# cropinghigh/sdrpp-dvbs-demodulator

Hardware: NVIDIA B200
Metric: decoded_info_gbit_s (higher is better)
Workload: dtype int8

## Files before the change

### sdrpp-dvbs-demodulator_b200/csrc/ldpc_decoder.cuh

```cuda
#pragma once
#include <cstdint>
#include <cuda_runtime.h>

namespace s2 {

constexpr int kLdpcThreads = 384;
constexpr int kBitWords = 13;
constexpr int16_t kLdpcItersNoInput = -2;

struct LdpcPlan;

struct LdpcDev {
    int N, K, R, q;
    int ngroups;
    int max_cnt;
    int sg;
    bool chains;
    bool occ3;
    bool v2;
    bool lanes2;
    const LdpcPlan* plan;
    const uint32_t* links;
    const int* layer_off;
    const uint8_t* layer_nlev;
    const uint8_t* row_level;
};
int ldpc_slot_groups(int max_cnt);
bool ldpc_chains_pay_off(int code_index);
bool ldpc_ctas_wanted3(int code_index);
bool ldpc_use_v2(int code_index);
bool ldpc_use_lanes2(int code_index);
int ldpc_slot_groups_for(int max_cnt, bool lanes2);
int ldpc_prepare(LdpcDev& code);
void ldpc_release(LdpcDev& code);

struct LdpcArgs {
    LdpcDev code;
    const int8_t* llr_in;
    int nframes;
    int max_trials;
    uint8_t* hard_out;
    int hard_stride;
    int16_t* iters_out;
    int8_t* llr_out;
    uint8_t* workspace;
    unsigned int* work_counter;
    const unsigned int* arrived;
};

inline size_t ldpc_workspace_bytes(const LdpcDev& c) {
    size_t b = (size_t)c.q * c.sg * 360 * 16 + (((size_t)c.R * 2 + 15) & ~(size_t)15);
    if (c.v2) b += (size_t)2 * (c.ngroups + c.q) * kBitWords * 4 + 32 + (size_t)768 * 16;
    return (b + 255) & ~(size_t)255;
}
inline size_t ldpc_smem_bytes(const LdpcDev& c) {
    if (c.v2 && c.lanes2) return (size_t)c.K * 2 + 768 + (size_t)c.q * (4 + 2 * ((2 * ((c.max_cnt + 1) / 2) + 3) & ~3)) * 4 + 64;
    if (c.v2) return (size_t)c.K * 2 + 768 + (size_t)c.q * ((1 + 2 * c.max_cnt + 3) & ~3) * 4 + 64;
    const size_t base = (size_t)c.K * 2 + (size_t)2 * (c.ngroups + c.q) * kBitWords * 4;
    return c.chains ? ((base + 15) & ~(size_t)15) + 360 * 16 + 64 : base + 64;
}

int ldpc_launch(const LdpcArgs& args, int grid, cudaStream_t stream);
int ldpc_max_ctas_per_sm(const LdpcDev& code);

}
```

### sdrpp-dvbs-demodulator_b200/csrc/ldpc_v2.cuh

```cuda
#pragma once
#include "ldpc_decoder.cuh"
#include "ldpc_variants.h"

#include <type_traits>

namespace s2 {
namespace v2 {

constexpr int kThreads = 360;

__device__ __forceinline__ uint32_t prmt(uint32_t a, uint32_t b, uint32_t sel) {
    uint32_t d;
    asm("prmt.b32 %0, %1, %2, %3;" : "=r"(d) : "r"(a), "r"(b), "r"(sel));
    return d;
}
__device__ __forceinline__ uint32_t minu2(uint32_t a, uint32_t b) {
    uint32_t d;
    asm("min.u16x2 %0, %1, %2;" : "=r"(d) : "r"(a), "r"(b));
    return d;
}
__device__ __forceinline__ uint32_t min3u2(uint32_t a, uint32_t b, uint32_t c) {
    uint32_t d;
    asm("{.reg .b32 t; min.u16x2 t, %1, %2; min.u16x2 %0, t, %3;}" : "=r"(d) : "r"(a), "r"(b), "r"(c));
    return d;
}
__device__ __forceinline__ uint32_t addmin_relu(uint32_t a, uint32_t b, uint32_t c) {
    uint32_t d;
    asm("{.reg .b32 t; add.s16x2 t, %1, %2; min.s16x2.relu %0, t, %3;}" : "=r"(d) : "r"(a), "r"(b), "r"(c));
    return d;
}
__device__ __forceinline__ uint32_t addmin(uint32_t a, uint32_t b, uint32_t c) {
    uint32_t d;
    asm("{.reg .b32 t; add.s16x2 t, %1, %2; min.s16x2 %0, t, %3;}" : "=r"(d) : "r"(a), "r"(b), "r"(c));
    return d;
}
__device__ __forceinline__ uint32_t addmin_u32(uint32_t x, uint32_t c) {
    uint32_t d;
    asm("{.reg .b32 t; add.u32 t, %1, %2; min.u32 %0, t, %1;}" : "=r"(d) : "r"(x), "r"(c));
    return d;
}
__device__ __forceinline__ uint32_t lds_u16(uint32_t addr) {
    uint16_t v;
    asm volatile("ld.shared.u16 %0, [%1];" : "=h"(v) : "r"(addr));
    return v;
}
__device__ __forceinline__ uint32_t lds_u32(uint32_t addr) {
    uint32_t v;
    asm volatile("ld.shared.u32 %0, [%1];" : "=r"(v) : "r"(addr));
    return v;
}
__device__ __forceinline__ void sts_u16(uint32_t addr, uint32_t v) {
    asm volatile("st.shared.u16 [%0], %1;" ::"r"(addr), "h"((uint16_t)v));
}

__device__ __forceinline__ uint32_t unpack_lo(uint32_t w) { return prmt(w, 0, 0x4140); }
__device__ __forceinline__ uint32_t unpack_hi(uint32_t w) { return prmt(w, 0, 0x4342); }
__device__ __forceinline__ uint32_t pack_pair(uint32_t x) { return prmt(x, 0, 0x4420); }
__device__ __forceinline__ uint32_t pack_two(uint32_t x0, uint32_t x1) { return prmt(x0, x1, 0x6420); }
__device__ __forceinline__ uint32_t lane_mask7(uint32_t x) { return prmt(x, 0, 0xAA88); }

constexpr uint32_t kC128 = 0x00800080u, kC255 = 0x00FF00FFu, kM32 = 0xFFE0FFE0u, kP32 = 0x00200020u;
constexpr uint32_t kP63 = 0x003F003Fu, kP64 = 0x00400040u, kAllOnes = 0xFFFFFFFFu;

template <int D>
__device__ __forceinline__ void exclusive_min(const uint32_t (&a)[D], uint32_t (&ex)[D]) {
    static_assert(D >= 3, "a check has at least three links");
    uint32_t P[D], S[D + 2];
#pragma unroll
    for (int i = 1; i < D; i += 2) P[i] = (i == 1) ? minu2(a[0], a[1]) : min3u2(P[i - 2], a[i - 1], a[i]);
    constexpr int top = (D & 1) ? D - 1 : D - 2;
    S[top] = (D & 1) ? a[D - 1] : minu2(a[D - 2], a[D - 1]);
#pragma unroll
    for (int i = top - 2; i >= 0; i -= 2) S[i] = min3u2(a[i], a[i + 1], S[i + 2]);
#pragma unroll
    for (int k = 0; k < D; ++k) {
        uint32_t t[4];
        int n = 0;
        if (k & 1) {
            if (k >= 3) t[n++] = P[k - 2];
            t[n++] = a[k - 1];
        } else if (k >= 2) {
            t[n++] = P[k - 1];
        }
        if (k + 1 <= D - 1) {
            if (((k + 1) & 1) == 0 && k + 1 <= top) {
                t[n++] = S[k + 1];
            } else {
                t[n++] = a[k + 1];
                if (k + 2 <= top) t[n++] = S[k + 2];
            }
        }
        ex[k] = (n == 1) ? t[0] : (n == 2) ? minu2(t[0], t[1]) : min3u2(t[0], t[1], t[2]);
    }
}

template <int CNT, bool FIRST, bool RAGGED>
__device__ __forceinline__ void row_update(const uint32_t (&off)[CNT], int cnt, uint32_t (&mw)[(CNT + 3) / 2],
                                           uint32_t& pown, uint32_t& psec, uint32_t keep, uint32_t m1) {
    constexpr int D = CNT + 2;
    uint32_t tu[D], a[D], ex[D];
    uint32_t sx = ((D - 1) & 1) ? kC128 : 0u;
#pragma unroll
    for (int c = 0; c < D; ++c) {
        uint32_t u;
        if (c < CNT)
            u = (!RAGGED || c < cnt) ? unpack_lo(lds_u16(off[c])) : kC255;
        else
            u = (c == CNT) ? pown : psec;
        uint32_t t = u;
        if (!FIRST) {
            const uint32_t beta = (c & 1) ? unpack_hi(mw[c >> 1]) : unpack_lo(mw[c >> 1]);
            t = addmin_relu(u + beta, kM32, kC255);
        }
        tu[c] = t;
        a[c] = __vabsdiffu4(t, kC128);
        sx ^= t;
    }
    exclusive_min<D>(a, ex);
    const uint32_t ssx = lane_mask7(sx);
    uint32_t prev = 0;
#pragma unroll
    for (int c = 0; c < D; ++c) {
        const uint32_t om = addmin_relu(ex[c], kAllOnes, kP32);
        const uint32_t neg = lane_mask7(tu[c]) ^ ssx;
        const uint32_t bias = neg * 0xFFFEFFFFu + kP32;
        const uint32_t bm = addmin(om ^ neg, bias, kP63);
        const uint32_t un = addmin_relu(tu[c] + bm, kM32, kC255);
        uint32_t beta;
        asm("mad.lo.u32 %0, %1, %2, %3;" : "=r"(beta) : "r"(bm), "r"(m1), "r"(kP64));
        if (c < CNT) {
            if (!RAGGED || c < cnt) sts_u16(off[c], pack_pair(un));
        } else if (c == CNT) {
            pown = un;
        } else {
            psec = un;
        }
        if (c & 1)
            mw[c >> 1] = pack_two(prev, beta);
        else if (c == D - 1)
            mw[c >> 1] = prmt(beta, keep, 0x7620);
        prev = beta;
    }
}


__device__ __forceinline__ uint32_t win360(const uint32_t* H, int o) {
    int w = o >> 5, s = o & 31;
    uint32_t r = __funnelshift_r(__ldcg(H + w), __ldcg(H + w + 1), s);
    int over = o + 32 - 360;
    if (over > 0) r |= __ldcg(H) << (32 - over);
    return r;
}
__device__ __forceinline__ uint32_t harvest8(uint4 w, uint32_t& nzacc) {
    const uint32_t k80 = 0x80808080u;
    nzacc &= __vabsdiffu4(w.x, k80) + 0x7F7F7F7Fu;
    nzacc &= __vabsdiffu4(w.y, k80) + 0x7F7F7F7Fu;
    nzacc &= __vabsdiffu4(w.z, k80) + 0x7F7F7F7Fu;
    nzacc &= __vabsdiffu4(w.w, k80) + 0x7F7F7F7Fu;
    uint32_t a0 = prmt(w.x, w.y, 0x6420), b0 = prmt(w.x, w.y, 0x7531);
    uint32_t a1 = prmt(w.z, w.w, 0x6420), b1 = prmt(w.z, w.w, 0x7531);
    auto mask4 = [](uint32_t x) { return (((~x & 0x80808080u) >> 7) * 0x00204081u >> 21) & 0xFu; };
    return mask4(a0) | (mask4(a1) << 4) | (mask4(b0) << 8) | (mask4(b1) << 12);
}
template <bool GLOBAL, int THREADS>
__device__ __forceinline__ void harvest_planes(const uint4* src, int n360, uint32_t* H, int gstride, int tid,
                                               uint32_t& nzacc) {
    uint8_t* Hb = reinterpret_cast<uint8_t*>(H);
    for (int t = tid; t < n360 * 45; t += THREADS) {
        uint4 w = GLOBAL ? __ldcg(src + t) : src[t];
        uint32_t bits = harvest8(w, nzacc);
        int g = t / 45, k = t - g * 45;
        __stcg(&Hb[g * (kBitWords * 4) + k], (uint8_t)bits);
        __stcg(&Hb[(gstride + g) * (kBitWords * 4) + k], (uint8_t)(bits >> 8));
    }
}

template <int THREADS>
__device__ __noinline__ int full_test(const LdpcParams2& p, const uint16_t* wpty, uint32_t* HP, uint32_t* HD,
                                      const uint4* vdata4, int* s_bad) {
    const int tid = threadIdx.x, q = p.q;
    uint32_t nzacc = 0xFFFFFFFFu;
    harvest_planes<true, THREADS>(reinterpret_cast<const uint4*>(wpty), q, HP, q, tid, nzacc);
    harvest_planes<false, THREADS>(vdata4, p.ngroups, HD, p.ngroups, tid, nzacc);
    if (tid < 2) s_bad[tid] = 0;
    __syncthreads();
    if (~nzacc & 0x00800080u) atomicOr(&s_bad[0], 1);
    if (~nzacc & 0x80008000u) atomicOr(&s_bad[1], 1);
    for (int task = tid; task < q * 12; task += THREADS) {
        const int ii = task / 12, w = task - ii * 12;
        const int loff = p.layer_off[ii], cnt = (int)p.layer_off[ii + 1] - loff;
        uint32_t sA = __ldcg(&HP[ii * kBitWords + w]), sB = __ldcg(&HP[(q + ii) * kBitWords + w]);
        if (ii > 0) {
            sA ^= __ldcg(&HP[(ii - 1) * kBitWords + w]);
            sB ^= __ldcg(&HP[(q + ii - 1) * kBitWords + w]);
        } else {
            const uint32_t* ta = &HP[(q - 1) * kBitWords];
            const uint32_t* tb = &HP[(2 * q - 1) * kBitWords];
            sA ^= (__ldcg(ta + w) << 1) | (w ? __ldcg(ta + w - 1) >> 31 : 0u);
            sB ^= (__ldcg(tb + w) << 1) | (w ? __ldcg(tb + w - 1) >> 31 : 0u);
        }
        for (int c = 0; c < cnt; ++c) {
            int o = 32 * w + (int)(p.link_add[loff + c] >> 1) - 360;
            o += (o < 0) ? 360 : 0;
            const int g = p.link_group[loff + c];
            sA ^= win360(&HD[g * kBitWords], o);
            sB ^= win360(&HD[(p.ngroups + g) * kBitWords], o);
        }
        if (w == 11) {
            sA &= 0xFFu;
            sB &= 0xFFu;
        }
        if (sA) atomicOr(&s_bad[0], 1);
        if (sB) atomicOr(&s_bad[1], 1);
    }
    __syncthreads();
    return (s_bad[0] ? 1 : 0) | (s_bad[1] ? 2 : 0);
}

template <int THREADS>
__device__ __noinline__ void emit_results(const LdpcParams2& p, int fin, const int (&res)[2], int fa, int fb,
                                          const uint16_t* wpty, const uint4* vdata4) {
    const int tid = threadIdx.x, q = p.q, K = p.K, N = p.N, R = p.R;
    const int kbytes = K / 8;
    for (int b = tid; b < kbytes; b += THREADS) {
        uint32_t nz = 0xFFFFFFFFu;
        const uint32_t bits = harvest8(vdata4[b], nz);
        if (fin & 1) p.hard_out[(size_t)fa * p.hard_stride + b] = (uint8_t)(__brev(bits & 0xFFu) >> 24);
        if (fin & 2) p.hard_out[(size_t)fb * p.hard_stride + b] = (uint8_t)(__brev((bits >> 8) & 0xFFu) >> 24);
    }
    for (int f = 0; f < 2; ++f) {
        if (!(fin >> f & 1)) continue;
        const int fr = f ? fb : fa;
        if (tid == 0) p.iters_out[fr] = (int16_t)res[f];
        if (p.llr_out) {
            int8_t* lo = p.llr_out + (size_t)fr * N;
            const uint8_t* vb = reinterpret_cast<const uint8_t*>(vdata4) + f;
            for (int x = tid; x < K; x += THREADS) lo[x] = (int8_t)(vb[2 * x] ^ 0x80u);
            for (int x = tid; x < R; x += THREADS) {
                const int jj = x / q, ii = x - jj * q;
                lo[K + x] = (int8_t)((__ldcg(&wpty[360 * ii + jj]) >> (8 * f)) ^ 0x80u);
            }
        }
    }
}

__device__ __forceinline__ uint4 interleave8(uint2 a, uint2 b) {
    uint4 o;
    o.x = prmt(a.x, b.x, 0x5140) ^ 0x80808080u;
    o.y = prmt(a.x, b.x, 0x7362) ^ 0x80808080u;
    o.z = prmt(a.y, b.y, 0x5140) ^ 0x80808080u;
    o.w = prmt(a.y, b.y, 0x7362) ^ 0x80808080u;
    return o;
}
template <bool STREAMED>
__device__ __forceinline__ uint2 ld_in8(const int8_t* frame, int x) {
    const uint2* s = reinterpret_cast<const uint2*>(frame) + x;
    return STREAMED ? __ldcg(s) : __ldg(s);
}

template <bool STREAMED, int THREADS>
__device__ __noinline__ void load_pair(const LdpcParams2& p, const int8_t* inA, const int8_t* inB, uint16_t* vdata,
                                       uint16_t* wpty) {
    static_assert(THREADS % 360 == 0, "a whole number of threads per column");
    const int tid = threadIdx.x, q = p.q, K = p.K;
    uint4* v4 = reinterpret_cast<uint4*>(vdata);
    const int8_t* ptA = inA + K;
    const int8_t* ptB = inB + K;
    const int cols = min(360, (K / q) & ~7);
    const int jj = tid % 360, i0 = tid / 360;
    for (int j0 = 0; j0 < 360; j0 += cols) {
        const int nc = min(cols, 360 - j0);
        const int b8 = q * j0 / 8;
        for (int x = tid; x < q * nc / 8; x += THREADS) v4[x] = interleave8(ld_in8<STREAMED>(ptA, b8 + x), ld_in8<STREAMED>(ptB, b8 + x));
        __syncthreads();
        if (jj < nc)
            for (int i = i0; i < q; i += THREADS / 360) __stcg(&wpty[i * 360 + j0 + jj], vdata[jj * q + i]);
        __syncthreads();
    }
    for (int x = tid; x < K / 8; x += THREADS) v4[x] = interleave8(ld_in8<STREAMED>(inA, x), ld_in8<STREAMED>(inB, x));
}

constexpr unsigned kNoPair = 0xFFFFFFFFu;
template <bool STREAMED>
__device__ __noinline__ unsigned claim_next_pair(const LdpcParams2& p, unsigned npairs) {
    if (*reinterpret_cast<const volatile unsigned*>(p.work_counter) + gridDim.x >= npairs) return kNoPair;
    const unsigned np = atomicAdd(p.work_counter, 1u);
    if (np < npairs) {
        const unsigned f0 = 2u * np, nf = min(2u, (unsigned)p.nframes - f0);
        if (!STREAMED || *reinterpret_cast<const volatile unsigned*>(p.arrived) >= f0 + nf) {
            const size_t b = reinterpret_cast<size_t>(p.llr_in + (size_t)f0 * p.N);
            const size_t lo = b & ~(size_t)15, hi = (b + (size_t)nf * p.N + 15) & ~(size_t)15;
            asm volatile("cp.async.bulk.prefetch.L2.global [%0], %1;" ::"l"(lo), "r"((unsigned)(hi - lo)) : "memory");
        }
    }
    return np;
}

static __device__ __noinline__ bool wait_arrived(const unsigned int* arrived_ptr, unsigned need, long long budget) {
    const volatile unsigned* arrived = arrived_ptr;
    const long long t0 = clock64();
    while (*arrived < need) {
        __nanosleep(500);
        if (clock64() - t0 > budget) return false;
    }
    return true;
}

template <int CNT, bool RAGGED, bool STREAMED, int OCC>
__global__ void __launch_bounds__(kThreads, OCC) ldpc_v2_kernel(const __grid_constant__ LdpcParams2 p) {
    constexpr int SLOTS = CNT + 2;
    constexpr int MW = (SLOTS + 1) / 2;
    constexpr int SG = (SLOTS + 7) / 8;
    static_assert(16 * SG >= 2 * SLOTS + 2, "the message record needs two spare bytes (row level)");
    constexpr int DW = (1 + 2 * CNT + 3) & ~3;
    extern __shared__ __align__(16) uint8_t smem_raw[];
    const int q = p.q, K = p.K, N = p.N, R = p.R;
    uint16_t* vdata = reinterpret_cast<uint16_t*>(smem_raw);
    uint16_t* X = reinterpret_cast<uint16_t*>(smem_raw + (size_t)K * 2);
    uint32_t* desc = reinterpret_cast<uint32_t*>(smem_raw + (size_t)K * 2 + 768);
    __shared__ unsigned int s_pair;
    __shared__ int s_bad[2];

    const int tid = threadIdx.x;
    const int j = tid;
    const uint32_t vbase = (uint32_t)__cvta_generic_to_shared(vdata);
    uint32_t dbase = (uint32_t)__cvta_generic_to_shared(desc);
    uint32_t j2 = 2u * (uint32_t)j;
    uint32_t xaddr = (uint32_t)__cvta_generic_to_shared(X) + j2;
    uint32_t m1 = 0xFFFFFFFFu;
    uint4* wmsg = reinterpret_cast<uint4*>(p.workspace + (size_t)blockIdx.x * p.ws_stride);
    uint16_t* wpty = reinterpret_cast<uint16_t*>(p.workspace + (size_t)blockIdx.x * p.ws_stride + (size_t)q * SG * 360 * 16);
    uint32_t* HD = reinterpret_cast<uint32_t*>(reinterpret_cast<uint8_t*>(wpty) + (((size_t)R * 2 + 15) & ~(size_t)15));
    uint32_t* HP = HD + 2 * p.ngroups * kBitWords;
    {
        volatile uint4* opq = reinterpret_cast<volatile uint4*>(HP + 2 * q * kBitWords + 4) + tid;
        opq->x = j2; opq->y = xaddr; opq->z = dbase; opq->w = m1;
        j2 = opq->x; xaddr = opq->y; dbase = opq->z; m1 = opq->w;
    }
    for (int x = tid; x < q * DW; x += kThreads) {
        const int i = x / DW, w = x - i * DW;
        const int loff = p.layer_off[i], cnt = (int)p.layer_off[i + 1] - loff;
        uint32_t v = 0;
        if (w == 0) {
            v = (uint32_t)p.layer_nlev[i] | (uint32_t)p.layer_sync[i] << 8 | (uint32_t)cnt << 16;
        } else if (w <= 2 * CNT) {
            const int c = (w - 1) >> 1;
            const int k = loff + (c < cnt ? c : 0);
            v = ((w - 1) & 1) ? (uint32_t)p.link_add[k] : vbase + 720u * p.link_group[k];
        }
        desc[x] = v;
    }
    const int npairs = (p.nframes + 1) >> 1;

    for (int x = tid; x < 2 * (p.ngroups + q) * kBitWords; x += kThreads) __stcg(&HD[x], 0u);
    __shared__ unsigned int s_next;
    if (tid == 0) s_next = kNoPair;

    for (;;) {
        __syncthreads();
        if (tid == 0) {
            unsigned np = s_next;
            if (np == kNoPair) np = atomicAdd(p.work_counter, 1u);
            s_next = kNoPair;
            if (STREAMED && np < (unsigned)npairs) {
                if (!wait_arrived(p.arrived, min(2u * np + 2u, (unsigned)p.nframes), p.wait_budget)) np |= 0x80000000u;
                __threadfence();
            }
            s_pair = np;
        }
        __syncthreads();
        const unsigned pair_word = s_pair;
        const unsigned pair = pair_word & 0x7FFFFFFFu;
        if (pair >= (unsigned)npairs) break;
        const int fa = 2 * pair, fb = 2 * pair + 1;
        const bool hasB = fb < p.nframes;
        if (STREAMED && (pair_word & 0x80000000u)) {
            if (tid == 0) {
                p.iters_out[fa] = kLdpcItersNoInput;
                if (hasB) p.iters_out[fb] = kLdpcItersNoInput;
            }
            continue;
        }
        const int8_t* inA = p.llr_in + (size_t)fa * N;
        const int8_t* inB = p.llr_in + (size_t)(hasB ? fb : fa) * N;

        load_pair<STREAMED, kThreads>(p, inA, inB, vdata, wpty);
        uint32_t pown = 0, psec = 0;
        {
            const uint32_t last = __ldcg(wpty + (q - 1) * 360 + j);
            X[j + 1] = (uint16_t)last;
            pown = unpack_lo(last);
            psec = unpack_lo(__ldcg(wpty + (q - 2) * 360 + j));
        }
        if (tid == 0) X[0] = 0xFFFFu;

        int live = hasB ? 3 : 1;
        uint32_t off[CNT];
        uint32_t lw0 = 0;
        auto link_addresses = [&](int i) {
            uint32_t dw[DW];
#pragma unroll
            for (int x = 0; x < DW; x += 4)
                asm volatile("ld.shared.v4.u32 {%0, %1, %2, %3}, [%4];" : "=r"(dw[x]), "=r"(dw[x + 1]), "=r"(dw[x + 2]), "=r"(dw[x + 3])
                             : "r"(dbase + (uint32_t)(i * DW + x) * 4u));
            lw0 = dw[0];
#pragma unroll
            for (int c = 0; c < CNT; ++c)
                off[c] = dw[1 + 2 * c] + addmin_u32(j2 + dw[2 + 2 * c], (uint32_t)-720);
        };
        auto screen = [&]() -> int {
            link_addresses(q - 1);
            const int cnt = (int)(lw0 >> 16);
            uint32_t sx = pown ^ psec, mn = minu2(__vabsdiffu4(pown, kC128), __vabsdiffu4(psec, kC128));
            int nl = 2;
#pragma unroll
            for (int c = 0; c < CNT; ++c) {
                if (!RAGGED || c < cnt) {
                    const uint32_t u = unpack_lo(lds_u16(off[c]));
                    sx ^= u;
                    mn = minu2(mn, __vabsdiffu4(u, kC128));
                    ++nl;
                }
            }
            if (nl & 1) sx ^= kC128;
            int bad = 0;
            if ((sx & 0x80u) || (mn & 0xFFFFu) == 0) bad |= 1;
            if ((sx & 0x800000u) || (mn >> 16) == 0) bad |= 2;
            return bad;
        };

        __syncthreads();
        int scr = screen();
        int res[2] = {-1, -1};
        for (int n = 0;; ++n) {
            int bad = (__syncthreads_or(scr & 1) ? 1 : 0) | (__syncthreads_or(scr & 2) ? 2 : 0);
            if (live & ~bad)
                bad = full_test<kThreads>(p, wpty, HP, HD, reinterpret_cast<const uint4*>(vdata), s_bad);
            int fin = 0;
            for (int f = 0; f < 2; ++f) {
                if (!(live >> f & 1)) continue;
                if (!(bad >> f & 1)) {
                    res[f] = n;
                    fin |= 1 << f;
                } else if (n == p.max_trials) {
                    fin |= 1 << f;
                }
            }
            if (fin) {
                emit_results<kThreads>(p, fin, res, fa, fb, wpty, reinterpret_cast<const uint4*>(vdata));
                if (tid == 0 && s_next == kNoPair) s_next = claim_next_pair<STREAMED>(p, (unsigned)npairs);
                live &= ~fin;
                if (live) __syncthreads();
            }
            if (!live) break;

            auto pass = [&](auto first_tag) {
                constexpr bool FIRST = decltype(first_tag)::value;
                uint32_t mw[MW];
                uint4 nxt[SG];
                uint32_t pnext = 0;
                uint32_t pprev = 0;
#pragma unroll
                for (int x = 0; x < MW; ++x) mw[x] = 0;
                uint4* rp = wmsg + j;
                uint16_t* pp = wpty + j;
                psec = unpack_lo(lds_u16(xaddr));
                pnext = __ldcg(pp);
                if (!FIRST) {
#pragma unroll
                    for (int s = 0; s < SG; ++s) nxt[s] = __ldcg(rp + s * 360);
                }
                uint32_t lev_next = (FIRST && p.layer_nlev[0] > 1) ? (uint32_t)p.row_level[j] << 24 : 0u;
                for (int i = 0; i < q; ++i) {
                    uint32_t keep = lev_next;
                    if (!FIRST) {
#pragma unroll
                        for (int s = 0; s < SG; ++s) {
                            if (4 * s + 0 < MW) mw[4 * s + 0] = nxt[s].x;
                            if (4 * s + 1 < MW) mw[4 * s + 1] = nxt[s].y;
                            if (4 * s + 2 < MW) mw[4 * s + 2] = nxt[s].z;
                            if (4 * s + 3 < MW) mw[4 * s + 3] = nxt[s].w;
                        }
                        keep = nxt[SG - 1].w;
                    }
                    pown = unpack_lo(i == q - 1 ? lds_u16(xaddr + 2) : pnext);
                    if (i + 1 < q) {
                        pnext = __ldcg(pp + 360);
                        if (!FIRST) {
#pragma unroll
                            for (int s = 0; s < SG; ++s) nxt[s] = __ldcg(rp + (SG + s) * 360);
                        }
                    }
                    link_addresses(i);
                    const int cnt = RAGGED ? (int)(lw0 >> 16) : CNT;
                    const int nlev = (int)(lw0 & 0xFFu);
                    if (FIRST) lev_next = (i + 1 < q && p.layer_nlev[i + 1] > 1) ? (uint32_t)p.row_level[(i + 1) * 360 + j] << 24 : 0u;
                    if (nlev == 1) {
                        row_update<CNT, FIRST, RAGGED>(off, cnt, mw, pown, psec, keep, m1);
                        if (lw0 & 0x100u) __syncthreads();
                    } else {
                        const int mylev = (int)(keep >> 24);
                        for (int lvl = 0; lvl < nlev; ++lvl) {
                            if (mylev == lvl) row_update<CNT, FIRST, RAGGED>(off, cnt, mw, pown, psec, keep, m1);
                            __syncthreads();
                        }
                    }
#pragma unroll
                    for (int s = 0; s < SG; ++s) {
                        uint4 o;
                        o.x = (4 * s + 0 < MW) ? mw[4 * s + 0] : 0u;
                        o.y = (4 * s + 1 < MW) ? mw[4 * s + 1] : 0u;
                        o.z = (4 * s + 2 < MW) ? mw[4 * s + 2] : 0u;
                        o.w = (4 * s + 3 < MW) ? mw[4 * s + 3] : 0u;
                        if (s == SG - 1 && 4 * s + 3 >= MW) o.w = keep & 0xFF000000u;
                        __stcg(rp + s * 360, o);
                    }
                    if (i == 0)
                        sts_u16(xaddr, pack_pair(psec));
                    else
                        __stcg(pp - 360, (uint16_t)pack_pair(psec));
                    pprev = psec;
                    psec = pown;
                    rp += SG * 360;
                    pp += 360;
                }
                psec = pprev;
                {
                    const uint16_t pk = (uint16_t)pack_pair(pown);
                    sts_u16(xaddr + 2, pk);
                    __stcg(pp - 360, pk);
                }
            };
            if (n == 0) pass(std::true_type{});
            else pass(std::false_type{});
            __syncthreads();
            scr = screen();
        }
    }
}

}
}

#define S2_V2_K4(c, r) {{v2::ldpc_v2_kernel<c, r, false, (c <= 9 ? 2 : 1)>, v2::ldpc_v2_kernel<c, r, false, (c <= 9 ? 3 : 2)>}, \
                        {v2::ldpc_v2_kernel<c, r, true, (c <= 9 ? 2 : 1)>, v2::ldpc_v2_kernel<c, r, true, (c <= 9 ? 3 : 2)>}}
#define S2_V2_N4 {{nullptr, nullptr}, {nullptr, nullptr}}
#define V2U(c) {c, S2_V2_K4(c, false), S2_V2_N4}
#define V2B(c) {c, S2_V2_K4(c, false), S2_V2_K4(c, true)}
#define V2R(c) {c, S2_V2_N4, S2_V2_K4(c, true)}
```

### sdrpp-dvbs-demodulator_b200/csrc/ldpc_v2l.cuh

```cuda
#pragma once
#include "ldpc_v2.cuh"

namespace s2 {
namespace v2 {

constexpr int kLdpcThreads2 = 720;

template <int NL, bool FIRST, bool RAGGED>
__device__ __forceinline__ void row_update2(const uint32_t (&off)[NL], int cntl, uint32_t (&mw)[(NL + 2) / 2], uint32_t& preg,
                                            uint32_t keep, uint32_t m1, unsigned lanes) {
    constexpr int DH = NL + 1;
    uint32_t tu[DH], a[DH];
    uint32_t sx = ((2 * DH - 1) & 1) ? kC128 : 0u;
#pragma unroll
    for (int s = 0; s < DH; ++s) {
        uint32_t u;
        if (s == 0)
            u = preg;
        else
            u = (!RAGGED || s - 1 < cntl) ? unpack_lo(lds_u16(off[s - 1])) : kC255;
        uint32_t t = u;
        if (!FIRST) {
            const uint32_t beta = (s & 1) ? unpack_hi(mw[s >> 1]) : unpack_lo(mw[s >> 1]);
            t = addmin_relu(u + beta, kM32, kC255);
        }
        tu[s] = t;
        a[s] = __vabsdiffu4(t, kC128);
        sx ^= t;
    }
    uint32_t P[DH], S[DH];
    P[0] = a[0];
#pragma unroll
    for (int s = 1; s < DH; ++s) P[s] = minu2(P[s - 1], a[s]);
    S[DH - 1] = a[DH - 1];
#pragma unroll
    for (int s = DH - 2; s >= 0; --s) S[s] = minu2(S[s + 1], a[s]);
    const uint32_t other = __shfl_xor_sync(lanes, P[DH - 1], 1);
    sx ^= __shfl_xor_sync(lanes, sx, 1) ^ (((2 * DH - 1) & 1) ? kC128 : 0u);
    const uint32_t ssx = lane_mask7(sx);
    uint32_t prev = 0;
#pragma unroll
    for (int s = 0; s < DH; ++s) {
        uint32_t ex;
        if (s == 0)
            ex = minu2(S[1], other);
        else if (s == DH - 1)
            ex = minu2(P[DH - 2], other);
        else
            ex = min3u2(P[s - 1], S[s + 1], other);
        const uint32_t om = addmin_relu(ex, kAllOnes, kP32);
        const uint32_t neg = lane_mask7(tu[s]) ^ ssx;
        const uint32_t bias = neg * 0xFFFEFFFFu + kP32;
        const uint32_t bm = addmin(om ^ neg, bias, kP63);
        const uint32_t un = addmin_relu(tu[s] + bm, kM32, kC255);
        uint32_t beta;
        asm("mad.lo.u32 %0, %1, %2, %3;" : "=r"(beta) : "r"(bm), "r"(m1), "r"(kP64));
        if (s == 0) {
            preg = un;
        } else if (!RAGGED || s - 1 < cntl) {
            sts_u16(off[s - 1], pack_pair(un));
        }
        if (s & 1)
            mw[s >> 1] = pack_two(prev, beta);
        else if (s == DH - 1)
            mw[s >> 1] = prmt(beta, keep, 0x7620);
        prev = beta;
    }
}

template <int CNT, bool RAGGED, bool STREAMED>
__global__ void __launch_bounds__(kLdpcThreads2, 1) ldpc_v2l_kernel(const __grid_constant__ LdpcParams2 p) {
    constexpr int T = kLdpcThreads2;
    constexpr int NL = (CNT + 1) / 2;
    constexpr int DH = NL + 1;
    constexpr int MW = (DH + 1) / 2;
    constexpr int SG = (DH + 7) / 8;
    static_assert(16 * SG >= 2 * DH + 2, "the message record needs two spare bytes (row level)");
    constexpr int HW = (2 * NL + 3) & ~3;
    constexpr int DW = 4 + 2 * HW;
    extern __shared__ __align__(16) uint8_t smem_raw[];
    const int q = p.q, K = p.K, N = p.N, R = p.R;
    uint16_t* vdata = reinterpret_cast<uint16_t*>(smem_raw);
    uint16_t* X = reinterpret_cast<uint16_t*>(smem_raw + (size_t)K * 2);
    uint32_t* desc = reinterpret_cast<uint32_t*>(smem_raw + (size_t)K * 2 + 768);
    __shared__ unsigned int s_pair;
    __shared__ int s_bad[2];

    const int tid = threadIdx.x;
    const int h = tid & 1;
    const int j = tid >> 1;
    const unsigned wl = __activemask();
    const int slot_t = 2 * j + h;
    const uint32_t vbase = (uint32_t)__cvta_generic_to_shared(vdata);
    uint32_t dbase = (uint32_t)__cvta_generic_to_shared(desc) + 16u + (uint32_t)h * HW * 4u;
    uint32_t j2 = 2u * (uint32_t)j;
    uint32_t xaddr = (uint32_t)__cvta_generic_to_shared(X) + j2;
    uint32_t m1 = 0xFFFFFFFFu;
    uint4* wmsg = reinterpret_cast<uint4*>(p.workspace + (size_t)blockIdx.x * p.ws_stride);
    uint16_t* wpty = reinterpret_cast<uint16_t*>(p.workspace + (size_t)blockIdx.x * p.ws_stride + (size_t)q * 2 * SG * 360 * 16);
    uint32_t* HD = reinterpret_cast<uint32_t*>(reinterpret_cast<uint8_t*>(wpty) + (((size_t)R * 2 + 15) & ~(size_t)15));
    uint32_t* HP = HD + 2 * p.ngroups * kBitWords;
    {
        volatile uint4* opq = reinterpret_cast<volatile uint4*>(HP + 2 * q * kBitWords + 4) + tid;
        opq->x = j2; opq->y = xaddr; opq->z = dbase; opq->w = m1;
        j2 = opq->x; xaddr = opq->y; dbase = opq->z; m1 = opq->w;
    }
    for (int x = tid; x < q * DW; x += T) {
        const int i = x / DW, w = x - i * DW;
        const int loff = p.layer_off[i], cnt = (int)p.layer_off[i + 1] - loff;
        uint32_t v = 0;
        if (w == 0) {
            v = (uint32_t)p.layer_nlev[i] | (uint32_t)p.layer_sync[i] << 8 | (uint32_t)cnt << 16;
        } else if (w >= 4) {
            const int hh = (w - 4) / HW, e = (w - 4) - hh * HW;
            const int s = e >> 1, d = 2 * s + hh;
            if (s < NL) {
                const int k = loff + (d < cnt ? d : 0);
                v = (e & 1) ? (uint32_t)p.link_add[k] : vbase + 720u * p.link_group[k];
            }
        }
        desc[x] = v;
    }
    const int npairs = (p.nframes + 1) >> 1;
    for (int x = tid; x < 2 * (p.ngroups + q) * kBitWords; x += T) __stcg(&HD[x], 0u);
    __shared__ unsigned int s_next;
    if (tid == 0) s_next = kNoPair;

    for (;;) {
        __syncthreads();
        if (tid == 0) {
            unsigned np = s_next;
            if (np == kNoPair) np = atomicAdd(p.work_counter, 1u);
            s_next = kNoPair;
            if (STREAMED && np < (unsigned)npairs) {
                if (!wait_arrived(p.arrived, min(2u * np + 2u, (unsigned)p.nframes), p.wait_budget)) np |= 0x80000000u;
                __threadfence();
            }
            s_pair = np;
        }
        __syncthreads();
        const unsigned pair_word = s_pair;
        const unsigned pair = pair_word & 0x7FFFFFFFu;
        if (pair >= (unsigned)npairs) break;
        const int fa = 2 * pair, fb = 2 * pair + 1;
        const bool hasB = fb < p.nframes;
        if (STREAMED && (pair_word & 0x80000000u)) {
            if (tid == 0) {
                p.iters_out[fa] = kLdpcItersNoInput;
                if (hasB) p.iters_out[fb] = kLdpcItersNoInput;
            }
            continue;
        }
        const int8_t* inA = p.llr_in + (size_t)fa * N;
        const int8_t* inB = p.llr_in + (size_t)(hasB ? fb : fa) * N;

        load_pair<STREAMED, T>(p, inA, inB, vdata, wpty);
        uint32_t preg;
        {
            const uint32_t w = __ldcg(wpty + (q - 1 - h) * 360 + j);
            if (h == 0) X[j + 1] = (uint16_t)w;
            preg = unpack_lo(w);
        }
        if (tid == 0) X[0] = 0xFFFFu;

        int live = hasB ? 3 : 1;
        uint32_t off[NL];
        uint32_t lw0 = 0;
        auto link_addresses = [&](int i) {
            uint32_t dw[HW];
            const uint32_t lb = dbase + (uint32_t)(i * DW) * 4u;
            lw0 = lds_u32(lb - 16u - (uint32_t)h * HW * 4u);
#pragma unroll
            for (int x = 0; x < HW; x += 4)
                asm volatile("ld.shared.v4.u32 {%0, %1, %2, %3}, [%4];" : "=r"(dw[x]), "=r"(dw[x + 1]), "=r"(dw[x + 2]), "=r"(dw[x + 3])
                             : "r"(lb + (uint32_t)x * 4u));
#pragma unroll
            for (int s = 0; s < NL; ++s) off[s] = dw[2 * s] + addmin_u32(j2 + dw[2 * s + 1], (uint32_t)-720);
        };
        auto half_links = [&](int cnt) { return (cnt - h + 1) >> 1; };
        auto screen = [&]() -> int {
            link_addresses(q - 1);
            const int cntl = half_links((int)(lw0 >> 16));
            uint32_t sx = preg, mn = __vabsdiffu4(preg, kC128);
            int nl = 1;
#pragma unroll
            for (int s = 0; s < NL; ++s) {
                if (s < cntl) {
                    const uint32_t u = unpack_lo(lds_u16(off[s]));
                    sx ^= u;
                    mn = minu2(mn, __vabsdiffu4(u, kC128));
                    ++nl;
                }
            }
            if (nl & 1) sx ^= kC128;
            sx ^= __shfl_xor_sync(wl, sx, 1);
            mn = minu2(mn, __shfl_xor_sync(wl, mn, 1));
            int bad = 0;
            if ((sx & 0x80u) || (mn & 0xFFFFu) == 0) bad |= 1;
            if ((sx & 0x800000u) || (mn >> 16) == 0) bad |= 2;
            return bad;
        };

        __syncthreads();
        int scr = screen();
        int res[2] = {-1, -1};
        for (int n = 0;; ++n) {
            int bad = (__syncthreads_or(scr & 1) ? 1 : 0) | (__syncthreads_or(scr & 2) ? 2 : 0);
            if (live & ~bad)
                bad = full_test<T>(p, wpty, HP, HD, reinterpret_cast<const uint4*>(vdata), s_bad);
            int fin = 0;
            for (int f = 0; f < 2; ++f) {
                if (!(live >> f & 1)) continue;
                if (!(bad >> f & 1)) {
                    res[f] = n;
                    fin |= 1 << f;
                } else if (n == p.max_trials) {
                    fin |= 1 << f;
                }
            }
            if (fin) {
                emit_results<T>(p, fin, res, fa, fb, wpty, reinterpret_cast<const uint4*>(vdata));
                if (tid == 0 && s_next == kNoPair) s_next = claim_next_pair<STREAMED>(p, (unsigned)npairs);
                live &= ~fin;
                if (live) __syncthreads();
            }
            if (!live) break;

            auto pass = [&](auto first_tag) {
                constexpr bool FIRST = decltype(first_tag)::value;
                uint32_t mw[MW];
                uint4 nxt[SG];
                uint32_t pnext = 0;
#pragma unroll
                for (int x = 0; x < MW; ++x) mw[x] = 0;
                uint4* rp = wmsg + slot_t;
                uint16_t* pp = wpty + j;
                if (h == 1) preg = unpack_lo(lds_u16(xaddr));
                pnext = __ldcg(pp);
                if (!FIRST) {
#pragma unroll
                    for (int s = 0; s < SG; ++s) nxt[s] = __ldcg(rp + s * 720);
                }
                uint32_t lev_next = (FIRST && p.layer_nlev[0] > 1) ? (uint32_t)p.row_level[j] << 24 : 0u;
                for (int i = 0; i < q; ++i) {
                    uint32_t keep = lev_next;
                    if (!FIRST) {
#pragma unroll
                        for (int s = 0; s < SG; ++s) {
                            if (4 * s + 0 < MW) mw[4 * s + 0] = nxt[s].x;
                            if (4 * s + 1 < MW) mw[4 * s + 1] = nxt[s].y;
                            if (4 * s + 2 < MW) mw[4 * s + 2] = nxt[s].z;
                            if (4 * s + 3 < MW) mw[4 * s + 3] = nxt[s].w;
                        }
                        keep = nxt[SG - 1].w;
                    }
                    if (h == 0)
                        preg = unpack_lo(i == q - 1 ? lds_u16(xaddr + 2) : pnext);
                    if (i + 1 < q) {
                        pnext = __ldcg(pp + 360);
                        if (!FIRST) {
#pragma unroll
                            for (int s = 0; s < SG; ++s) nxt[s] = __ldcg(rp + (SG + s) * 720);
                        }
                    }
                    link_addresses(i);
                    const int cntl = RAGGED ? half_links((int)(lw0 >> 16)) : (h == 0 ? (CNT + 1) / 2 : CNT / 2);
                    const int nlev = (int)(lw0 & 0xFFu);
                    if (FIRST) lev_next = (i + 1 < q && p.layer_nlev[i + 1] > 1) ? (uint32_t)p.row_level[(i + 1) * 360 + j] << 24 : 0u;
                    constexpr bool kPartial = RAGGED || (CNT & 1);
                    if (nlev == 1) {
                        row_update2<NL, FIRST, kPartial>(off, cntl, mw, preg, keep, m1, wl);
                        if (lw0 & 0x100u) __syncthreads();
                    } else {
                        const int mylev = (int)(keep >> 24);
                        for (int lvl = 0; lvl < nlev; ++lvl) {
                            const unsigned lanes = __ballot_sync(wl, mylev == lvl);
                            if (mylev == lvl) row_update2<NL, FIRST, kPartial>(off, cntl, mw, preg, keep, m1, lanes);
                            __syncthreads();
                        }
                    }
#pragma unroll
                    for (int s = 0; s < SG; ++s) {
                        uint4 o;
                        o.x = (4 * s + 0 < MW) ? mw[4 * s + 0] : 0u;
                        o.y = (4 * s + 1 < MW) ? mw[4 * s + 1] : 0u;
                        o.z = (4 * s + 2 < MW) ? mw[4 * s + 2] : 0u;
                        o.w = (4 * s + 3 < MW) ? mw[4 * s + 3] : 0u;
                        if (s == SG - 1 && (4 * s + 3 >= MW || !(DH & 1))) o.w = (o.w & 0x00FFFFFFu) | (keep & 0xFF000000u);
                        __stcg(rp + s * 720, o);
                    }
                    if (h == 1) {
                        if (i == 0)
                            sts_u16(xaddr, pack_pair(preg));
                        else
                            __stcg(pp - 360, (uint16_t)pack_pair(preg));
                    }
                    const uint32_t other = __shfl_xor_sync(wl, preg, 1);
                    if (h == 1 && i + 1 < q) preg = other;
                    rp += 2 * SG * 360;
                    pp += 360;
                }
                if (h == 0) {
                    const uint16_t pk = (uint16_t)pack_pair(preg);
                    sts_u16(xaddr + 2, pk);
                    __stcg(pp - 360, pk);
                }
            };
            if (n == 0) pass(std::true_type{});
            else pass(std::false_type{});
            __syncthreads();
            scr = screen();
        }
    }
}

}
}

#define S2_V2L_K2(c, r) {v2::ldpc_v2l_kernel<c, r, false>, v2::ldpc_v2l_kernel<c, r, true>}
#define S2_V2L_N2 {nullptr, nullptr}
#define V2LU(c) {c, S2_V2L_K2(c, false), S2_V2L_N2}
#define V2LR(c) {c, S2_V2L_N2, S2_V2L_K2(c, true)}
```

Measured before the change: 23.69.

## Move LDPC full syndrome test bit-planes into shared memory with warp-shuffle parity

The full parity check no longer harvests hard-decision bit planes for both data and parity into a global workspace. It builds a per-frame data plane in shared memory and derives the parity-chain XOR on the fly using warp shuffles over loads from the parity buffer. Only frames still undecided after the screen are tested, and the per-layer link loop is unrolled by the CNT template. This drops the global plane stores and reloads, the atomic bad flags, and the workspace zeroing. In exchange it uses extra shared memory per block, which may lower occupancy, and runs the two frames sequentially with extra syncs.

```diff
diff --git a/sdrpp-dvbs-demodulator_b200/csrc/ldpc_decoder.cuh b/sdrpp-dvbs-demodulator_b200/csrc/ldpc_decoder.cuh
--- a/sdrpp-dvbs-demodulator_b200/csrc/ldpc_decoder.cuh
+++ b/sdrpp-dvbs-demodulator_b200/csrc/ldpc_decoder.cuh
@@ -50,12 +50,13 @@
 
 inline size_t ldpc_workspace_bytes(const LdpcDev& c) {
     size_t b = (size_t)c.q * c.sg * 360 * 16 + (((size_t)c.R * 2 + 15) & ~(size_t)15);
-    if (c.v2) b += (size_t)2 * (c.ngroups + c.q) * kBitWords * 4 + 32 + (size_t)768 * 16;
+    if (c.v2) b += (size_t)768 * 16;
     return (b + 255) & ~(size_t)255;
 }
 inline size_t ldpc_smem_bytes(const LdpcDev& c) {
-    if (c.v2 && c.lanes2) return (size_t)c.K * 2 + 768 + (size_t)c.q * (4 + 2 * ((2 * ((c.max_cnt + 1) / 2) + 3) & ~3)) * 4 + 64;
-    if (c.v2) return (size_t)c.K * 2 + 768 + (size_t)c.q * ((1 + 2 * c.max_cnt + 3) & ~3) * 4 + 64;
+    const size_t plane = (size_t)c.ngroups * kBitWords * 4;
+    if (c.v2 && c.lanes2) return (size_t)c.K * 2 + 768 + (size_t)c.q * (4 + 2 * ((2 * ((c.max_cnt + 1) / 2) + 3) & ~3)) * 4 + plane + 64;
+    if (c.v2) return (size_t)c.K * 2 + 768 + (size_t)c.q * ((1 + 2 * c.max_cnt + 3) & ~3) * 4 + plane + 64;
     const size_t base = (size_t)c.K * 2 + (size_t)2 * (c.ngroups + c.q) * kBitWords * 4;
     return c.chains ? ((base + 15) & ~(size_t)15) + 360 * 16 + 64 : base + 64;
 }
diff --git a/sdrpp-dvbs-demodulator_b200/csrc/ldpc_v2.cuh b/sdrpp-dvbs-demodulator_b200/csrc/ldpc_v2.cuh
--- a/sdrpp-dvbs-demodulator_b200/csrc/ldpc_v2.cuh
+++ b/sdrpp-dvbs-demodulator_b200/csrc/ldpc_v2.cuh
@@ -144,13 +144,6 @@
 }
 
 
-__device__ __forceinline__ uint32_t win360(const uint32_t* H, int o) {
-    int w = o >> 5, s = o & 31;
-    uint32_t r = __funnelshift_r(__ldcg(H + w), __ldcg(H + w + 1), s);
-    int over = o + 32 - 360;
-    if (over > 0) r |= __ldcg(H) << (32 - over);
-    return r;
-}
 __device__ __forceinline__ uint32_t harvest8(uint4 w, uint32_t& nzacc) {
     const uint32_t k80 = 0x80808080u;
     nzacc &= __vabsdiffu4(w.x, k80) + 0x7F7F7F7Fu;
@@ -162,59 +155,84 @@
     auto mask4 = [](uint32_t x) { return (((~x & 0x80808080u) >> 7) * 0x00204081u >> 21) & 0xFu; };
     return mask4(a0) | (mask4(a1) << 4) | (mask4(b0) << 8) | (mask4(b1) << 12);
 }
-template <bool GLOBAL, int THREADS>
-__device__ __forceinline__ void harvest_planes(const uint4* src, int n360, uint32_t* H, int gstride, int tid,
-                                               uint32_t& nzacc) {
-    uint8_t* Hb = reinterpret_cast<uint8_t*>(H);
-    for (int t = tid; t < n360 * 45; t += THREADS) {
-        uint4 w = GLOBAL ? __ldcg(src + t) : src[t];
-        uint32_t bits = harvest8(w, nzacc);
-        int g = t / 45, k = t - g * 45;
-        __stcg(&Hb[g * (kBitWords * 4) + k], (uint8_t)bits);
-        __stcg(&Hb[(gstride + g) * (kBitWords * 4) + k], (uint8_t)(bits >> 8));
-    }
-}
-
-template <int THREADS>
-__device__ __noinline__ int full_test(const LdpcParams2& p, const uint16_t* wpty, uint32_t* HP, uint32_t* HD,
-                                      const uint4* vdata4, int* s_bad) {
-    const int tid = threadIdx.x, q = p.q;
-    uint32_t nzacc = 0xFFFFFFFFu;
-    harvest_planes<true, THREADS>(reinterpret_cast<const uint4*>(wpty), q, HP, q, tid, nzacc);
-    harvest_planes<false, THREADS>(vdata4, p.ngroups, HD, p.ngroups, tid, nzacc);
-    if (tid < 2) s_bad[tid] = 0;
-    __syncthreads();
-    if (~nzacc & 0x00800080u) atomicOr(&s_bad[0], 1);
-    if (~nzacc & 0x80008000u) atomicOr(&s_bad[1], 1);
-    for (int task = tid; task < q * 12; task += THREADS) {
-        const int ii = task / 12, w = task - ii * 12;
-        const int loff = p.layer_off[ii], cnt = (int)p.layer_off[ii + 1] - loff;
-        uint32_t sA = __ldcg(&HP[ii * kBitWords + w]), sB = __ldcg(&HP[(q + ii) * kBitWords + w]);
-        if (ii > 0) {
-            sA ^= __ldcg(&HP[(ii - 1) * kBitWords + w]);
-            sB ^= __ldcg(&HP[(q + ii - 1) * kBitWords + w]);
-        } else {
-            const uint32_t* ta = &HP[(q - 1) * kBitWords];
-            const uint32_t* tb = &HP[(2 * q - 1) * kBitWords];
-            sA ^= (__ldcg(ta + w) << 1) | (w ? __ldcg(ta + w - 1) >> 31 : 0u);
-            sB ^= (__ldcg(tb + w) << 1) | (w ? __ldcg(tb + w - 1) >> 31 : 0u);
-        }
-        for (int c = 0; c < cnt; ++c) {
-            int o = 32 * w + (int)(p.link_add[loff + c] >> 1) - 360;
-            o += (o < 0) ? 360 : 0;
-            const int g = p.link_group[loff + c];
-            sA ^= win360(&HD[g * kBitWords], o);
-            sB ^= win360(&HD[(p.ngroups + g) * kBitWords], o);
-        }
-        if (w == 11) {
-            sA &= 0xFFu;
-            sB &= 0xFFu;
-        }
-        if (sA) atomicOr(&s_bad[0], 1);
-        if (sB) atomicOr(&s_bad[1], 1);
-    }
-    __syncthreads();
-    return (s_bad[0] ? 1 : 0) | (s_bad[1] ? 2 : 0);
+template <int THREADS, int CNT, bool RAGGED>
+__device__ __noinline__ int full_test(const LdpcParams2& p, const uint16_t* wpty, const uint4* vdata4, uint32_t* plane,
+                                      int cand) {
+    const int tid = threadIdx.x, lane = tid & 31, q = p.q;
+    const int nchunks = (q + 31) >> 5;
+    const int li = lane >> 2, qd = lane & 3;
+    int bad = 0;
+    for (int f = 0; f < 2; ++f) {
+        if (!(cand >> f & 1)) continue;
+        const int sh = 8 * f;
+        uint32_t nz = 0xFFFFFFFFu;
+        for (int t = tid; t < p.ngroups * kBitWords; t += THREADS) {
+            const int g = t / kBitWords, w = t - g * kBitWords;
+            uint32_t word = 0;
+#pragma unroll
+            for (int k = 0; k < 4; ++k) {
+                int x = 4 * w + k;
+                x -= (x >= 45) ? 45 : 0;
+                word |= ((harvest8(vdata4[g * 45 + x], nz) >> sh) & 0xFFu) << (8 * k);
+            }
+            plane[t] = word;
+        }
+        __syncthreads();
+        const uint32_t pbase = (uint32_t)__cvta_generic_to_shared(plane);
+        int fbad = 0;
+        for (int b = tid >> 5; b < 12 * nchunks && (tid | 31) < THREADS; b += THREADS / 32) {
+            const int w = b % 12, i0 = 32 * (b / 12);
+            const int r8 = 32 * w + 8 * qd;
+            auto ld8 = [&](int i) -> uint4 {
+                return (r8 < 360 && i < q) ? __ldcg(reinterpret_cast<const uint4*>(wpty + i * 360 + r8))
+                                           : make_uint4(~0u, ~0u, ~0u, ~0u);
+            };
+            auto word_of = [&](const uint4 v) {
+                uint32_t x = ((harvest8(v, nz) >> sh) & 0xFFu) << (8 * qd);
+                x |= __shfl_xor_sync(0xFFFFFFFFu, x, 1);
+                return x | __shfl_xor_sync(0xFFFFFFFFu, x, 2);
+            };
+            uint32_t below = word_of(ld8(i0 > 0 ? i0 - 1 : q - 1));
+            if (i0 == 0) {
+                const uint32_t c = w > 0 ? (~(uint32_t)__ldcg(wpty + (q - 1) * 360 + 32 * w - 1) >> (7 + sh)) & 1u : 0u;
+                below = (below << 1) | c;
+            }
+            uint32_t mine = 0;
+            uint4 v[2];
+#pragma unroll
+            for (int k = 0; k < 4; ++k) {
+                if (!(k & 1)) {
+                    v[0] = ld8(i0 + 8 * k + li);
+                    v[1] = ld8(i0 + 8 * k + 8 + li);
+                }
+                const uint32_t wk = word_of(v[k & 1]);
+                const uint32_t dn = __shfl_sync(0xFFFFFFFFu, wk, (lane - 4) & 31);
+                const uint32_t check = wk ^ (li > 0 ? dn : below);
+                const uint32_t t = __shfl_sync(0xFFFFFFFFu, check, (lane & 7) * 4);
+                if ((lane >> 3) == k) mine = t;
+                below = __shfl_sync(0xFFFFFFFFu, wk, 28 + qd);
+            }
+            const int i = i0 + lane;
+            if (i < q) {
+                const int loff = p.layer_off[i], cnt = (int)p.layer_off[i + 1] - loff;
+                uint32_t s = mine;
+#pragma unroll
+                for (int c = 0; c < CNT; ++c) {
+                    if (!RAGGED || c < cnt) {
+                        int o = 32 * w + (int)(p.link_add[loff + c] >> 1) - 360;
+                        o += (o < 0) ? 360 : 0;
+                        const uint32_t a = pbase + (uint32_t)(p.link_group[loff + c] * kBitWords + (o >> 5)) * 4u;
+                        s ^= __funnelshift_r(lds_u32(a), lds_u32(a + 4), o & 31);
+                    }
+                }
+                if (w == 11) s &= 0xFFu;
+                fbad |= s != 0;
+            }
+        }
+        fbad |= (~nz & (0x00800080u << sh)) != 0;
+        bad |= __syncthreads_or(fbad) ? 1 << f : 0;
+    }
+    return bad;
 }
 
 template <int THREADS>
@@ -318,8 +336,8 @@
     uint16_t* vdata = reinterpret_cast<uint16_t*>(smem_raw);
     uint16_t* X = reinterpret_cast<uint16_t*>(smem_raw + (size_t)K * 2);
     uint32_t* desc = reinterpret_cast<uint32_t*>(smem_raw + (size_t)K * 2 + 768);
+    uint32_t* plane = desc + q * DW;
     __shared__ unsigned int s_pair;
-    __shared__ int s_bad[2];
 
     const int tid = threadIdx.x;
     const int j = tid;
@@ -330,10 +348,8 @@
     uint32_t m1 = 0xFFFFFFFFu;
     uint4* wmsg = reinterpret_cast<uint4*>(p.workspace + (size_t)blockIdx.x * p.ws_stride);
     uint16_t* wpty = reinterpret_cast<uint16_t*>(p.workspace + (size_t)blockIdx.x * p.ws_stride + (size_t)q * SG * 360 * 16);
-    uint32_t* HD = reinterpret_cast<uint32_t*>(reinterpret_cast<uint8_t*>(wpty) + (((size_t)R * 2 + 15) & ~(size_t)15));
-    uint32_t* HP = HD + 2 * p.ngroups * kBitWords;
     {
-        volatile uint4* opq = reinterpret_cast<volatile uint4*>(HP + 2 * q * kBitWords + 4) + tid;
+        volatile uint4* opq = reinterpret_cast<volatile uint4*>(reinterpret_cast<uint8_t*>(wpty) + (((size_t)R * 2 + 15) & ~(size_t)15)) + tid;
         opq->x = j2; opq->y = xaddr; opq->z = dbase; opq->w = m1;
         j2 = opq->x; xaddr = opq->y; dbase = opq->z; m1 = opq->w;
     }
@@ -352,7 +368,6 @@
     }
     const int npairs = (p.nframes + 1) >> 1;
 
-    for (int x = tid; x < 2 * (p.ngroups + q) * kBitWords; x += kThreads) __stcg(&HD[x], 0u);
     __shared__ unsigned int s_next;
     if (tid == 0) s_next = kNoPair;
 
@@ -434,8 +449,8 @@
         int res[2] = {-1, -1};
         for (int n = 0;; ++n) {
             int bad = (__syncthreads_or(scr & 1) ? 1 : 0) | (__syncthreads_or(scr & 2) ? 2 : 0);
-            if (live & ~bad)
-                bad = full_test<kThreads>(p, wpty, HP, HD, reinterpret_cast<const uint4*>(vdata), s_bad);
+            if (const int cand = live & ~bad)
+                bad |= full_test<kThreads, CNT, RAGGED>(p, wpty, reinterpret_cast<const uint4*>(vdata), plane, cand);
             int fin = 0;
             for (int f = 0; f < 2; ++f) {
                 if (!(live >> f & 1)) continue;
diff --git a/sdrpp-dvbs-demodulator_b200/csrc/ldpc_v2l.cuh b/sdrpp-dvbs-demodulator_b200/csrc/ldpc_v2l.cuh
--- a/sdrpp-dvbs-demodulator_b200/csrc/ldpc_v2l.cuh
+++ b/sdrpp-dvbs-demodulator_b200/csrc/ldpc_v2l.cuh
@@ -83,8 +83,8 @@
     uint16_t* vdata = reinterpret_cast<uint16_t*>(smem_raw);
     uint16_t* X = reinterpret_cast<uint16_t*>(smem_raw + (size_t)K * 2);
     uint32_t* desc = reinterpret_cast<uint32_t*>(smem_raw + (size_t)K * 2 + 768);
+    uint32_t* plane = desc + q * DW;
     __shared__ unsigned int s_pair;
-    __shared__ int s_bad[2];
 
     const int tid = threadIdx.x;
     const int h = tid & 1;
@@ -98,10 +98,8 @@
     uint32_t m1 = 0xFFFFFFFFu;
     uint4* wmsg = reinterpret_cast<uint4*>(p.workspace + (size_t)blockIdx.x * p.ws_stride);
     uint16_t* wpty = reinterpret_cast<uint16_t*>(p.workspace + (size_t)blockIdx.x * p.ws_stride + (size_t)q * 2 * SG * 360 * 16);
-    uint32_t* HD = reinterpret_cast<uint32_t*>(reinterpret_cast<uint8_t*>(wpty) + (((size_t)R * 2 + 15) & ~(size_t)15));
-    uint32_t* HP = HD + 2 * p.ngroups * kBitWords;
     {
-        volatile uint4* opq = reinterpret_cast<volatile uint4*>(HP + 2 * q * kBitWords + 4) + tid;
+        volatile uint4* opq = reinterpret_cast<volatile uint4*>(reinterpret_cast<uint8_t*>(wpty) + (((size_t)R * 2 + 15) & ~(size_t)15)) + tid;
         opq->x = j2; opq->y = xaddr; opq->z = dbase; opq->w = m1;
         j2 = opq->x; xaddr = opq->y; dbase = opq->z; m1 = opq->w;
     }
@@ -122,7 +120,6 @@
         desc[x] = v;
     }
     const int npairs = (p.nframes + 1) >> 1;
-    for (int x = tid; x < 2 * (p.ngroups + q) * kBitWords; x += T) __stcg(&HD[x], 0u);
     __shared__ unsigned int s_next;
     if (tid == 0) s_next = kNoPair;
 
@@ -206,8 +203,8 @@
         int res[2] = {-1, -1};
         for (int n = 0;; ++n) {
             int bad = (__syncthreads_or(scr & 1) ? 1 : 0) | (__syncthreads_or(scr & 2) ? 2 : 0);
-            if (live & ~bad)
-                bad = full_test<T>(p, wpty, HP, HD, reinterpret_cast<const uint4*>(vdata), s_bad);
+            if (const int cand = live & ~bad)
+                bad |= full_test<T, CNT, RAGGED>(p, wpty, reinterpret_cast<const uint4*>(vdata), plane, cand);
             int fin = 0;
             for (int f = 0; f < 2; ++f) {
                 if (!(live >> f & 1)) continue;
```

New measurement: 23.25 (median of 6 runs). 1.9% lower.
